# miaoyin390/DNN-Compression-Tensor-ADMM

Measured on AMD Instinct MI355X. Metric: ADMM projection iters/sec (all layers) + per-layer SVD GFLOP/s, ResNet-50 TT ranks, higher is better.
Workload: dtype f32 (Gram, eigen-solve and its filter products accumulate in f64); 1 GPU; resnet50_tt: 34 layers, 20099072 weights, hp table tt_resnet50_hp.HyperParamsDictGeneralRatio3x; tables=1, parallelism=layer-shard x1 (latency-model partition, one scalar all-reduce per step)

## Files before the change

### dnn-compression-tensor-admm_amd/csrc/dgemm.hip

```cpp
#include "common.h"

namespace tadmm {

typedef double double4_t __attribute__((ext_vector_type(4)));
typedef double double2_t __attribute__((ext_vector_type(2)));

struct DgemmArgs {
  const double *A, *B, *C, *P, *Q;
  double *ring0, *ring1, *ring2;
  const int32_t* rot;
  int32_t selA, selB, selC, selP, selQ;
  int32_t M, N, K, lda, ldb, ldc, tiles_m, tiles_n, mode;
  const double* coef; const double* theta; double* rowpart;
  const int32_t* gate; int32_t gate_min;
};
__device__ __forceinline__ DgemmArgs dg_args(const DgemmDesc* __restrict__ g) {
  DgemmArgs d;
  d.A = g->A; d.B = g->B; d.C = g->C; d.P = g->P; d.Q = g->Q;
  d.ring0 = g->ring[0]; d.ring1 = g->ring[1]; d.ring2 = g->ring[2];
  d.rot = g->rot;
  d.selA = g->selA; d.selB = g->selB; d.selC = g->selC; d.selP = g->selP; d.selQ = g->selQ;
  d.M = g->M; d.N = g->N; d.K = g->K; d.lda = g->lda; d.ldb = g->ldb; d.ldc = g->ldc;
  d.tiles_m = g->tiles_m; d.tiles_n = g->tiles_n; d.mode = g->mode;
  d.coef = g->coef; d.theta = g->theta; d.rowpart = g->rowpart;
  d.gate = g->gate; d.gate_min = g->gate_min;
  return d;
}

__device__ __forceinline__ const double* dg_sel(const DgemmArgs& d, int sel, const double* explicit_ptr, int base) {
  if (sel < 0) return explicit_ptr;
  int i = base + sel;
  i -= (i >= 3) ? 3 : 0;
  i -= (i >= 3) ? 3 : 0;
  const double* r0 = +d.ring0; const double* r1 = +d.ring1; const double* r2 = +d.ring2;
  return i == 0 ? +r0 : (i == 1 ? +r1 : +r2);
}

#ifdef TADMM_DGEMM_STAMPS
__device__ long long g_dstamps[64];
#define DSTAMP(i) do { if (blockIdx.x == 0 && threadIdx.x == 0) g_dstamps[i] = (long long)__builtin_readcyclecounter(); } while (0)
#else
#define DSTAMP(i) do { } while (0)
#endif

template <bool kBT>
__global__ __launch_bounds__(256) void dgemm_kernel(const DgemmDesc* __restrict__ descs,
                                                    const BlockRef* __restrict__ map) {
  __shared__ double red[4][4][64 * 4];
  __shared__ double rowred[32][33];
  const BlockRef br = map[blockIdx.x];
  const DgemmArgs d = dg_args(descs + br.prob);
  if (d.gate && *d.gate < d.gate_min) return;
  const int base = d.rot ? *d.rot : 0;
  const double* __restrict__ A = dg_sel(d, d.selA, d.A, base);
  const double* __restrict__ B = dg_sel(d, d.selB, d.B, base);
  double* __restrict__ C = const_cast<double*>(dg_sel(d, d.selC, d.C, base));
  const int tm = br.local / d.tiles_n, tn = br.local - tm * d.tiles_n;
  const int lane = threadIdx.x & 63, wave = threadIdx.x >> 6;
  const int r = lane & 15, q = lane >> 4;
  const int K = d.K;
  const int per = (((K + 3) / 4) + 15) & ~15;
  const int wk0 = min(K, wave * per), wk1 = min(K, wk0 + per);

  double4_t acc00 = {0, 0, 0, 0}, acc01 = {0, 0, 0, 0}, acc10 = {0, 0, 0, 0}, acc11 = {0, 0, 0, 0};
  const int64_t lda = d.lda, ldb = d.ldb;
  const double* pa0 = A + (int64_t)(tm * 32 + r) * lda;
  const double* pa1 = pa0 + 16 * lda;

  struct Chunk { double a0[4], a1[4], b0[4], b1[4]; };
  auto mma = [&](const Chunk& c) {
#pragma unroll
    for (int e = 0; e < 4; ++e) {
      acc00 = __builtin_amdgcn_mfma_f64_16x16x4f64(c.a0[e], c.b0[e], acc00, 0, 0, 0);
      acc01 = __builtin_amdgcn_mfma_f64_16x16x4f64(c.a0[e], c.b1[e], acc01, 0, 0, 0);
      acc10 = __builtin_amdgcn_mfma_f64_16x16x4f64(c.a1[e], c.b0[e], acc10, 0, 0, 0);
      acc11 = __builtin_amdgcn_mfma_f64_16x16x4f64(c.a1[e], c.b1[e], acc11, 0, 0, 0);
    }
  };
  auto fetch = [&](int kk, Chunk& c) {
    const int k = kk + 4 * q;
    const double2_t t0 = *reinterpret_cast<const double2_t*>(pa0 + k), t1 = *reinterpret_cast<const double2_t*>(pa0 + k + 2);
    const double2_t t2 = *reinterpret_cast<const double2_t*>(pa1 + k), t3 = *reinterpret_cast<const double2_t*>(pa1 + k + 2);
    c.a0[0] = t0.x; c.a0[1] = t0.y; c.a0[2] = t1.x; c.a0[3] = t1.y;
    c.a1[0] = t2.x; c.a1[1] = t2.y; c.a1[2] = t3.x; c.a1[3] = t3.y;
    if (kBT) {
      const double* pb0 = B + (int64_t)(tn * 32 + r) * ldb + k;
      const double* pb1 = pb0 + 16 * ldb;
      const double2_t u0 = *reinterpret_cast<const double2_t*>(pb0), u1 = *reinterpret_cast<const double2_t*>(pb0 + 2);
      const double2_t u2 = *reinterpret_cast<const double2_t*>(pb1), u3 = *reinterpret_cast<const double2_t*>(pb1 + 2);
      c.b0[0] = u0.x; c.b0[1] = u0.y; c.b0[2] = u1.x; c.b0[3] = u1.y;
      c.b1[0] = u2.x; c.b1[1] = u2.y; c.b1[2] = u3.x; c.b1[3] = u3.y;
    } else {
      const double* pb = B + (int64_t)k * ldb + tn * 32 + r;
#pragma unroll
      for (int e = 0; e < 4; ++e) { c.b0[e] = pb[(int64_t)e * ldb]; c.b1[e] = pb[(int64_t)e * ldb + 16]; }
    }
  };
  if (wk0 < wk1) {
    Chunk cur, nxt;
    fetch(wk0, cur);
    for (int kk = wk0; kk < wk1; kk += 16) {
      const bool more = kk + 16 < wk1;
      if (more) fetch(kk + 16, nxt);
      mma(cur);
      if (more) cur = nxt;
    }
  }
#pragma unroll
  for (int e = 0; e < 4; ++e) {
    red[wave][0][lane * 4 + e] = acc00[e];
    red[wave][1][lane * 4 + e] = acc01[e];
    red[wave][2][lane * 4 + e] = acc10[e];
    red[wave][3][lane * 4 + e] = acc11[e];
  }
  __syncthreads();
  const int mode = d.mode;
  double s0 = 1.0, s1 = 0.0, s2 = 0.0;
  if (mode == 1) { s0 = d.coef[0]; s1 = d.coef[1]; s2 = d.coef[2]; }
  const double* __restrict__ P = (mode >= 1) ? dg_sel(d, d.selP, d.P, base) : nullptr;
  const double* __restrict__ Q = (mode == 1 && s2 != 0.0) ? dg_sel(d, d.selQ, d.Q, base) : nullptr;
  const int64_t ldc = d.ldc;
  {
    const int row = threadIdx.x >> 3, c4 = (threadIdx.x & 7) * 4;
    double v[4];
#pragma unroll
    for (int u = 0; u < 4; ++u) {
      const int col = c4 + u;
      const int t = ((row >> 4) << 1) | (col >> 4);
      const int rr = row & 15, cc = col & 15;
      const int le = ((((rr & 3) << 4) | cc) << 2) | (rr >> 2);
      v[u] = (red[0][t][le] + red[1][t][le]) + (red[2][t][le] + red[3][t][le]);
    }
    const int64_t gi = (int64_t)(tm * 32 + row) * ldc + tn * 32 + c4;
    if (mode == 0) {
      *reinterpret_cast<double2_t*>(C + gi) = double2_t{v[0], v[1]};
      *reinterpret_cast<double2_t*>(C + gi + 2) = double2_t{v[2], v[3]};
    } else if (mode == 1) {
      const double2_t p0 = *reinterpret_cast<const double2_t*>(P + gi), p1 = *reinterpret_cast<const double2_t*>(P + gi + 2);
      double o[4] = {s0 * v[0] + s1 * p0.x, s0 * v[1] + s1 * p0.y, s0 * v[2] + s1 * p1.x, s0 * v[3] + s1 * p1.y};
      if (Q) {
        const double2_t q0 = *reinterpret_cast<const double2_t*>(Q + gi), q1 = *reinterpret_cast<const double2_t*>(Q + gi + 2);
        o[0] += s2 * q0.x; o[1] += s2 * q0.y; o[2] += s2 * q1.x; o[3] += s2 * q1.y;
      }
      *reinterpret_cast<double2_t*>(C + gi) = double2_t{o[0], o[1]};
      *reinterpret_cast<double2_t*>(C + gi + 2) = double2_t{o[2], o[3]};
    } else {
      const double2_t p0 = *reinterpret_cast<const double2_t*>(P + gi), p1 = *reinterpret_cast<const double2_t*>(P + gi + 2);
      double part;
      if (mode == 2) {
        *reinterpret_cast<double2_t*>(C + gi) = double2_t{v[0], v[1]};
        *reinterpret_cast<double2_t*>(C + gi + 2) = double2_t{v[2], v[3]};
        part = (v[0] * p0.x + v[1] * p0.y) + (v[2] * p1.x + v[3] * p1.y);
      } else {
        const double th = d.theta[tm * 32 + row];
        const double e0 = v[0] - th * p0.x, e1 = v[1] - th * p0.y, e2 = v[2] - th * p1.x, e3 = v[3] - th * p1.y;
        part = (e0 * e0 + e1 * e1) + (e2 * e2 + e3 * e3);
      }
      rowred[row][threadIdx.x & 7] = part;
    }
  }
  if (mode >= 2) {
    __syncthreads();
    if (threadIdx.x < 32) {
      const double* p = rowred[threadIdx.x];
      d.rowpart[(int64_t)tn * d.M + tm * 32 + threadIdx.x] = ((p[0] + p[1]) + (p[2] + p[3])) + ((p[4] + p[5]) + (p[6] + p[7]));
    }
  }
}

void launch_dgemm(const DgemmDesc* descs_dev, const BlockRef* map_dev, int nblocks, bool b_transposed, hipStream_t s) {
  if (nblocks <= 0) return;
  if (b_transposed) hipLaunchKernelGGL(dgemm_kernel<true>, dim3(nblocks), dim3(256), 0, s, descs_dev, map_dev);
  else hipLaunchKernelGGL(dgemm_kernel<false>, dim3(nblocks), dim3(256), 0, s, descs_dev, map_dev);
}


constexpr int kDT = 64, kDK = 32, kDLd = kDK + 2;

template <int TN, int KW, int TM = kDT>
__global__ __launch_bounds__(128 * (TM / 32) * KW) void dgemm_nt_tile_kernel(const DgemmDesc* __restrict__ descs,
                                                                            const BlockRef* __restrict__ map) {
  constexpr int NT = 128 * (TM / 32) * KW;
  constexpr int WN = TN / 2;
  constexpr int NB = WN / 16;
  constexpr int AP = TM * 16 / NT;
  constexpr int BP = TN * 16 / NT;
  constexpr int RS = NT / 16;
  constexpr int TPR = 256 / TM;
  constexpr int CPT = TN / TPR;
  constexpr int kBuf = (TM + TN) * kDLd;
  static_assert(AP >= 1 && BP >= 1 && CPT >= 2, "tile / thread layout");
  __shared__ __attribute__((aligned(16))) double smem[2 * kBuf > TM * (TN + 1) ? 2 * kBuf : TM * (TN + 1)];
  __shared__ double rowred[TM][TPR];
  const BlockRef br = map[blockIdx.x];
  const DgemmArgs d = dg_args(descs + br.prob);
  if (d.gate && *d.gate < d.gate_min) return;
  const int base = d.rot ? *d.rot : 0;
  const G<const double>* __restrict__ A = gp(dg_sel(d, d.selA, d.A, base));
  const G<const double>* __restrict__ B = gp(dg_sel(d, d.selB, d.B, base));
  G<double>* __restrict__ C = gp(const_cast<double*>(dg_sel(d, d.selC, d.C, base)));
  const int tiles_n = (d.N + TN - 1) / TN;
  const int tm = br.local / tiles_n, tn = br.local - tm * tiles_n;
  const int m0 = tm * TM, n0 = tn * TN;
  const int tid = threadIdx.x, lane = tid & 63, wave = tid >> 6;
  const int r = lane & 15, q = lane >> 4;
  const int kh = (TM == 64) ? wave >> 2 : wave >> 1, wm = (TM == 64) ? (wave >> 1) & 1 : 0, wn = wave & 1;
  const int K = d.K;
  const int64_t lda = d.lda, ldb = d.ldb;
  const bool live = (m0 + 32 * wm < d.M) && (n0 + WN * wn < d.N);

  struct Regs { double2_t a[AP], b[BP]; };
  const int srow = tid >> 4, sc2 = tid & 15;
  const G<const double>* pa[AP]; const G<const double>* pb[BP];
#pragma unroll
  for (int i = 0; i < AP; ++i) pa[i] = A + (int64_t)min(m0 + srow + RS * i, d.M - 1) * lda + 2 * sc2;
#pragma unroll
  for (int i = 0; i < BP; ++i) pb[i] = B + (int64_t)min(n0 + srow + RS * i, d.N - 1) * ldb + 2 * sc2;
  auto gload = [&](Regs& R, int k0) {
#pragma unroll
    for (int i = 0; i < AP; ++i) R.a[i] = *reinterpret_cast<const G<const double2_t>*>(pa[i] + k0);
#pragma unroll
    for (int i = 0; i < BP; ++i) R.b[i] = *reinterpret_cast<const G<const double2_t>*>(pb[i] + k0);
  };
  auto sstore = [&](const Regs& R, int stage) {
    double (*As)[kDLd] = reinterpret_cast<double (*)[kDLd]>(smem + stage * kBuf);
    double (*Bs)[kDLd] = As + TM;
#pragma unroll
    for (int i = 0; i < AP; ++i) *reinterpret_cast<double2_t*>(&As[srow + RS * i][2 * sc2]) = R.a[i];
#pragma unroll
    for (int i = 0; i < BP; ++i) *reinterpret_cast<double2_t*>(&Bs[srow + RS * i][2 * sc2]) = R.b[i];
  };
  double4_t acc[2][NB];
#pragma unroll
  for (int i = 0; i < 2; ++i)
#pragma unroll
    for (int j = 0; j < NB; ++j) acc[i][j] = double4_t{0, 0, 0, 0};
  auto compute = [&](int stage) {
    if (!live) return;
    const double (*As)[kDLd] = reinterpret_cast<const double (*)[kDLd]>(smem + stage * kBuf);
    const double (*Bs)[kDLd] = As + TM;
    const int kof = kh * (kDK / KW);
    const double* a0p = &As[32 * wm + r][q + kof];
    const double* a1p = &As[32 * wm + 16 + r][q + kof];
    const double* b0p = &Bs[WN * wn + r][q + kof];
    constexpr int KS = kDK / KW / 4;
    double fa0[KS], fa1[KS], fb[KS][NB];
#pragma unroll
    for (int s = 0; s < KS; ++s) {
      fa0[s] = a0p[4 * s]; fa1[s] = a1p[4 * s];
#pragma unroll
      for (int j = 0; j < NB; ++j) fb[s][j] = b0p[16 * j * kDLd + 4 * s];
    }
#pragma unroll
    for (int s = 0; s < KS; ++s) {
#pragma unroll
      for (int j = 0; j < NB; ++j) {
        acc[0][j] = __builtin_amdgcn_mfma_f64_16x16x4f64(fa0[s], fb[s][j], acc[0][j], 0, 0, 0);
        acc[1][j] = __builtin_amdgcn_mfma_f64_16x16x4f64(fa1[s], fb[s][j], acc[1][j], 0, 0, 0);
      }
    }
  };
  DSTAMP(0);
  const int nch = K / kDK;
  constexpr int NPF = 2;
  Regs R[NPF];
#pragma unroll
  for (int u = 0; u < NPF; ++u)
    if (u < nch) gload(R[u], u * kDK);
  sstore(R[0], 0);
  if (NPF < nch) gload(R[0], NPF * kDK);
  __syncthreads();
  DSTAMP(1);
  for (int c = 0; c < nch; c += NPF) {
#pragma unroll
    for (int u = 0; u < NPF; ++u) {
      const int i = c + u;
      if (i < nch) {
        if (i + 1 < nch) {
          sstore(R[(u + 1) % NPF], (u + 1) & 1);
          if (i + 1 + NPF < nch) gload(R[(u + 1) % NPF], (i + 1 + NPF) * kDK);
        }
        compute(u & 1);
        DSTAMP(2 + 2 * i);
        __syncthreads();
        DSTAMP(3 + 2 * i);
      }
    }
  }
  double (*Ct)[TN + 1] = reinterpret_cast<double (*)[TN + 1]>(smem);
#pragma unroll
  for (int h = KW - 1; h >= 0; --h) {
    if (kh == h) {
#pragma unroll
      for (int e = 0; e < 4; ++e)
#pragma unroll
        for (int i = 0; i < 2; ++i)
#pragma unroll
          for (int j = 0; j < NB; ++j) {
            double* c = &Ct[32 * wm + 16 * i + q + 4 * e][WN * wn + 16 * j + r];
            *c = (h == KW - 1 ? 0.0 : *c) + acc[i][j][e];
          }
    }
    __syncthreads();
  }
  if (NT > 256 && tid >= 256) return;
  const int mode = d.mode;
  double s0 = 1.0, s1 = 0.0, s2 = 0.0;
  if (mode == 1) { s0 = d.coef[0]; s1 = d.coef[1]; s2 = d.coef[2]; }
  const G<const double>* __restrict__ P = gp((mode >= 1) ? dg_sel(d, d.selP, d.P, base) : nullptr);
  const G<const double>* __restrict__ Q = gp((mode == 1 && s2 != 0.0) ? dg_sel(d, d.selQ, d.Q, base) : nullptr);
  const int64_t ldc = d.ldc;
  const int row = tid / TPR, c0 = (tid % TPR) * CPT;
  const bool rok = m0 + row < d.M;
  double part = 0.0;
  if (rok && n0 + c0 < d.N) {
    const double th = (mode == 3) ? d.theta[m0 + row] : 0.0;
#pragma unroll
    for (int u = 0; u < CPT; u += 2) {
      const int col = c0 + u;
      const int64_t gi = (int64_t)(m0 + row) * ldc + n0 + col;
      const double v0 = Ct[row][col], v1 = Ct[row][col + 1];
      if (mode == 0) {
        *reinterpret_cast<G<double2_t>*>(C + gi) = double2_t{v0, v1};
      } else {
        const double2_t p = *reinterpret_cast<const G<const double2_t>*>(P + gi);
        if (mode == 1) {
          double o0 = s0 * v0 + s1 * p.x, o1 = s0 * v1 + s1 * p.y;
          if (Q) {
            const double2_t qq = *reinterpret_cast<const G<const double2_t>*>(Q + gi);
            o0 += s2 * qq.x; o1 += s2 * qq.y;
          }
          *reinterpret_cast<G<double2_t>*>(C + gi) = double2_t{o0, o1};
        } else if (mode == 2) {
          *reinterpret_cast<G<double2_t>*>(C + gi) = double2_t{v0, v1};
          part += v0 * p.x + v1 * p.y;
        } else {
          const double e0 = v0 - th * p.x, e1 = v1 - th * p.y;
          part += e0 * e0 + e1 * e1;
        }
      }
    }
  }
  DSTAMP(40);
  if (mode >= 2) {
    rowred[row][tid % TPR] = part;
    __syncthreads();
    if (tid < TM && m0 + tid < d.M) {
      const double* pr = rowred[tid];
      double sum = (pr[0] + pr[1]) + (pr[2] + pr[3]);
      if (TPR == 8) sum += (pr[4] + pr[5]) + (pr[6] + pr[7]);
      d.rowpart[(int64_t)tn * d.M + m0 + tid] = sum;
    }
  }
}

void launch_dgemm_nt64(const DgemmDesc* descs_dev, const BlockRef* map_dev, int nblocks, hipStream_t s, int tile_n, int tile_m) {
  if (nblocks <= 0) return;
#ifdef TADMM_DGEMM_STAMPS
  if (getenv("TADMM_DGEMM_STAMPS_DUMP")) {
    long long h[64];
    (void)hipDeviceSynchronize();
    (void)hipMemcpyFromSymbol(h, HIP_SYMBOL(g_dstamps), sizeof h);
    fprintf(stderr, "[dgemm stamps]");
    for (int i = 1; i < 41; ++i) if (h[i]) fprintf(stderr, " %d:%lld", i, h[i] - h[0]);
    fprintf(stderr, "\n");
  }
#endif
  static const int kw = getenv("TADMM_DGEMM_KW") ? atoi(getenv("TADMM_DGEMM_KW")) : 2;
  if (tile_m == 32) {
    hipLaunchKernelGGL((dgemm_nt_tile_kernel<32, 4, 32>), dim3(nblocks), dim3(512), 0, s, descs_dev, map_dev);
    return;
  }
  if (tile_n == 32) {
    if (kw == 2) hipLaunchKernelGGL((dgemm_nt_tile_kernel<32, 2>), dim3(nblocks), dim3(512), 0, s, descs_dev, map_dev);
    else hipLaunchKernelGGL((dgemm_nt_tile_kernel<32, 1>), dim3(nblocks), dim3(256), 0, s, descs_dev, map_dev);
  } else {
    if (kw == 2) hipLaunchKernelGGL((dgemm_nt_tile_kernel<64, 2>), dim3(nblocks), dim3(512), 0, s, descs_dev, map_dev);
    else hipLaunchKernelGGL((dgemm_nt_tile_kernel<64, 1>), dim3(nblocks), dim3(256), 0, s, descs_dev, map_dev);
  }
}

__global__ __launch_bounds__(256) void daxpby_kernel(const DgemmDesc* __restrict__ descs, const BlockRef* __restrict__ map) {
  const BlockRef br = map[blockIdx.x];
  const DgemmArgs d = dg_args(descs + br.prob);
  if (d.gate && *d.gate < d.gate_min) return;
  const int base = d.rot ? *d.rot : 0;
  double* __restrict__ C = const_cast<double*>(dg_sel(d, d.selC, d.C, base));
  const double* __restrict__ P = dg_sel(d, d.selP, d.P, base);
  const double s0 = d.coef[0], s1 = d.coef[1];
  const int64_t total = (int64_t)d.M * d.ldc;
  const int64_t i0 = ((int64_t)br.local * 256 + threadIdx.x) * 4;
  if (i0 + 3 < total) {
    const double2_t c0 = *reinterpret_cast<const double2_t*>(C + i0), c1 = *reinterpret_cast<const double2_t*>(C + i0 + 2);
    const double2_t p0 = *reinterpret_cast<const double2_t*>(P + i0), p1 = *reinterpret_cast<const double2_t*>(P + i0 + 2);
    *reinterpret_cast<double2_t*>(C + i0) = double2_t{s0 * c0.x + s1 * p0.x, s0 * c0.y + s1 * p0.y};
    *reinterpret_cast<double2_t*>(C + i0 + 2) = double2_t{s0 * c1.x + s1 * p1.x, s0 * c1.y + s1 * p1.y};
  } else {
    for (int64_t i = i0; i < total; ++i) C[i] = s0 * C[i] + s1 * P[i];
  }
}

void launch_daxpby(const DgemmDesc* descs_dev, const BlockRef* map_dev, int nblocks, hipStream_t s) {
  if (nblocks <= 0) return;
  hipLaunchKernelGGL(daxpby_kernel, dim3(nblocks), dim3(256), 0, s, descs_dev, map_dev);
}

}
```

Before: 164.8 iters/s.

## Prefetch epilogue operands early and fold split-K partials in parallel

The DGEMM tile kernel now fetches descriptor scalars, gate, rotation and coefficients up front. It also issues the epilogue loads for P, Q and theta before or after the K loop, so their latency overlaps with the MFMA work. The serial per-kh shared-memory reduction, which needed KW barriers, is replaced by each k-slice writing its own shared buffer and the epilogue threads summing the slices. This trades extra LDS capacity (KW times the C tile) and more live registers, which may cut occupancy, for fewer barriers and hidden global latency.

```diff
diff --git a/dnn-compression-tensor-admm_amd/csrc/dgemm.hip b/dnn-compression-tensor-admm_amd/csrc/dgemm.hip
--- a/dnn-compression-tensor-admm_amd/csrc/dgemm.hip
+++ b/dnn-compression-tensor-admm_amd/csrc/dgemm.hip
@@ -190,12 +190,25 @@
   constexpr int CPT = TN / TPR;
   constexpr int kBuf = (TM + TN) * kDLd;
   static_assert(AP >= 1 && BP >= 1 && CPT >= 2, "tile / thread layout");
-  __shared__ __attribute__((aligned(16))) double smem[2 * kBuf > TM * (TN + 1) ? 2 * kBuf : TM * (TN + 1)];
+  __shared__ __attribute__((aligned(16))) double smem[2 * kBuf > KW * TM * (TN + 1) ? 2 * kBuf : KW * TM * (TN + 1)];
   __shared__ double rowred[TM][TPR];
   const BlockRef br = map[blockIdx.x];
-  const DgemmArgs d = dg_args(descs + br.prob);
-  if (d.gate && *d.gate < d.gate_min) return;
-  const int base = d.rot ? *d.rot : 0;
+  const DgemmDesc* __restrict__ gd = descs + br.prob;
+  const DgemmArgs d = dg_args(gd);
+  asm volatile("" ::"s"(d.A), "s"(d.B), "s"(d.C), "s"(d.P), "s"(d.Q), "s"(d.ring0), "s"(d.ring1), "s"(d.ring2));
+  asm volatile("" ::"s"(d.selA), "s"(d.selB), "s"(d.selC), "s"(d.selP), "s"(d.selQ), "s"(d.M), "s"(d.N), "s"(d.K),
+               "s"(d.lda), "s"(d.ldb), "s"(d.ldc), "s"(d.theta), "s"(d.rowpart));
+  const int mode = d.mode;
+  const int32_t* dword = &gd->gate_min;
+  const int gate_v = *gp(d.gate ? d.gate : dword);
+  const int rot_v = *gp(d.rot ? d.rot : dword);
+  const G<const double>* cf = gp((mode == 1) ? d.coef : reinterpret_cast<const double*>(gd));
+  const double cf0 = cf[0], cf1 = cf[1], cf2 = cf[2];
+  asm volatile("" ::"v"(gate_v), "v"(rot_v), "v"(cf0), "v"(cf1), "v"(cf2));
+  if (d.gate && gate_v < d.gate_min) return;
+  const int base = d.rot ? rot_v : 0;
+  double s0 = 1.0, s1 = 0.0, s2 = 0.0;
+  if (mode == 1) { s0 = cf0; s1 = cf1; s2 = cf2; }
   const G<const double>* __restrict__ A = gp(dg_sel(d, d.selA, d.A, base));
   const G<const double>* __restrict__ B = gp(dg_sel(d, d.selB, d.B, base));
   G<double>* __restrict__ C = gp(const_cast<double*>(dg_sel(d, d.selC, d.C, base)));
@@ -267,6 +280,27 @@
 #pragma unroll
   for (int u = 0; u < NPF; ++u)
     if (u < nch) gload(R[u], u * kDK);
+  const G<const double>* __restrict__ P = gp((mode >= 1) ? dg_sel(d, d.selP, d.P, base) : nullptr);
+  const G<const double>* __restrict__ Q = gp((mode == 1 && s2 != 0.0) ? dg_sel(d, d.selQ, d.Q, base) : nullptr);
+  const int64_t ldc = d.ldc;
+  const int row = tid / TPR, c0 = (tid % TPR) * CPT;
+  const bool rok = m0 + row < d.M;
+  const bool mine = (NT == 256 || tid < 256) && rok && n0 + c0 < d.N;
+  const int64_t gi0 = (int64_t)(m0 + row) * ldc + n0 + c0;
+  const G<const double>* ppre = (mine && P) ? P + gi0 : A;
+  const G<const double>* qpre = (mine && Q) ? Q + gi0 : A;
+  const G<const double>* tpre = (mine && mode == 3) ? gp(d.theta) + (m0 + row) : A;
+  double2_t pp[CPT / 2], pq[CPT / 2];
+  double th_pre;
+  auto fetch_epilogue = [&]() {
+#pragma unroll
+    for (int u = 0; u < CPT / 2; ++u) pp[u] = *reinterpret_cast<const G<const double2_t>*>(ppre + 2 * u);
+#pragma unroll
+    for (int u = 0; u < CPT / 2; ++u) pq[u] = *reinterpret_cast<const G<const double2_t>*>(qpre + 2 * u);
+    th_pre = *tpre;
+  };
+  constexpr bool kEpiEarly = CPT <= 8;
+  if (kEpiEarly) fetch_epilogue();
   sstore(R[0], 0);
   if (NPF < nch) gload(R[0], NPF * kDK);
   __syncthreads();
@@ -287,47 +321,38 @@
       }
     }
   }
-  double (*Ct)[TN + 1] = reinterpret_cast<double (*)[TN + 1]>(smem);
-#pragma unroll
-  for (int h = KW - 1; h >= 0; --h) {
-    if (kh == h) {
-#pragma unroll
-      for (int e = 0; e < 4; ++e)
-#pragma unroll
-        for (int i = 0; i < 2; ++i)
-#pragma unroll
-          for (int j = 0; j < NB; ++j) {
-            double* c = &Ct[32 * wm + 16 * i + q + 4 * e][WN * wn + 16 * j + r];
-            *c = (h == KW - 1 ? 0.0 : *c) + acc[i][j][e];
-          }
-    }
-    __syncthreads();
-  }
+  if (!kEpiEarly) fetch_epilogue();
+  double (*Ct)[TM][TN + 1] = reinterpret_cast<double (*)[TM][TN + 1]>(smem);
+#pragma unroll
+  for (int e = 0; e < 4; ++e)
+#pragma unroll
+    for (int i = 0; i < 2; ++i)
+#pragma unroll
+      for (int j = 0; j < NB; ++j) Ct[kh][32 * wm + 16 * i + q + 4 * e][WN * wn + 16 * j + r] = acc[i][j][e];
+  __syncthreads();
   if (NT > 256 && tid >= 256) return;
-  const int mode = d.mode;
-  double s0 = 1.0, s1 = 0.0, s2 = 0.0;
-  if (mode == 1) { s0 = d.coef[0]; s1 = d.coef[1]; s2 = d.coef[2]; }
-  const G<const double>* __restrict__ P = gp((mode >= 1) ? dg_sel(d, d.selP, d.P, base) : nullptr);
-  const G<const double>* __restrict__ Q = gp((mode == 1 && s2 != 0.0) ? dg_sel(d, d.selQ, d.Q, base) : nullptr);
-  const int64_t ldc = d.ldc;
-  const int row = tid / TPR, c0 = (tid % TPR) * CPT;
-  const bool rok = m0 + row < d.M;
+  auto folded = [&](int rr, int cc) {
+    double v = 0.0 + Ct[KW - 1][rr][cc];
+#pragma unroll
+    for (int h = KW - 2; h >= 0; --h) v = v + Ct[h][rr][cc];
+    return v;
+  };
   double part = 0.0;
   if (rok && n0 + c0 < d.N) {
-    const double th = (mode == 3) ? d.theta[m0 + row] : 0.0;
+    const double th = (mode == 3) ? th_pre : 0.0;
 #pragma unroll
     for (int u = 0; u < CPT; u += 2) {
       const int col = c0 + u;
       const int64_t gi = (int64_t)(m0 + row) * ldc + n0 + col;
-      const double v0 = Ct[row][col], v1 = Ct[row][col + 1];
+      const double v0 = folded(row, col), v1 = folded(row, col + 1);
       if (mode == 0) {
         *reinterpret_cast<G<double2_t>*>(C + gi) = double2_t{v0, v1};
       } else {
-        const double2_t p = *reinterpret_cast<const G<const double2_t>*>(P + gi);
+        const double2_t p = pp[u / 2];
         if (mode == 1) {
           double o0 = s0 * v0 + s1 * p.x, o1 = s0 * v1 + s1 * p.y;
           if (Q) {
-            const double2_t qq = *reinterpret_cast<const G<const double2_t>*>(Q + gi);
+            const double2_t qq = pq[u / 2];
             o0 += s2 * qq.x; o1 += s2 * qq.y;
           }
           *reinterpret_cast<G<double2_t>*>(C + gi) = double2_t{o0, o1};
```

After: 166.0 iters/s, median of 6. Within noise of the previous version (+0.8%).
